# oscarknagg/voicemap

Measured on AMD Instinct MI355X. Metric: audio-sec/s embedded, 3s@16kHz siamese batch (training step), higher is better.
Workload: dtype f16; 1 GPU; siamese cfg-A train step (filters 128, embed 64, contrastive loss), 128 pairs/GPU of 3 s @ 16 kHz decimated x4 (L=12000), Adam(clipnorm 1), f16 storage; global_pairs=128, parallelism=dp1

## Files before the change

voicemap_amd/csrc/conv_wgrad.hip:

```cpp
#include "conv_common.hpp"

namespace vm {

template <typename T>
struct TnArgs {
    const T* x;
    const T* du;
    float* ws;
    int64_t x_win_stride, du_win_stride;
    int c_in, c_out, L;
    int Kk;
    int tilesI, tilesJ, splits;
    int xcd_remap;
    int64_t n_windows, win_per_split;
    int split = 0;
    int64_t tower_windows = 0;
    int splits_per_tower = 0;
    int64_t stages_per_split = 0;
};

template <typename T>
__device__ inline void split_windows(const TnArgs<T>& p, int split, int64_t& w_begin, int64_t& w_end) {
    const int tw = split / p.splits_per_tower, j = split - tw * p.splits_per_tower;
    const int64_t t0 = (int64_t)tw * p.tower_windows;
    int64_t t1 = t0 + p.tower_windows;
    if (t1 > p.n_windows) t1 = p.n_windows;
    w_begin = t0 + (int64_t)j * p.win_per_split;
    w_end = w_begin + p.win_per_split;
    if (w_end > t1) w_end = t1;
    if (w_begin > w_end) w_begin = w_end;
}

template <typename T, int PITCH, int SZ = (int)sizeof(T)> struct Transpose4;
template <typename T, int PITCH> struct Transpose4<T, PITCH, 2> {
    __device__ static inline void store(char* lds_tile, int col0, int pg, const u32x4 (&v)[4]) {
#pragma unroll
        for (int j = 0; j < 8; ++j) {
            const uint32_t sel = (j & 1) ? 0x07060302u : 0x05040100u;
            u32x2 o;
            o[0] = __builtin_amdgcn_perm(v[1][j >> 1], v[0][j >> 1], sel);
            o[1] = __builtin_amdgcn_perm(v[3][j >> 1], v[2][j >> 1], sel);
            *reinterpret_cast<u32x2*>(lds_tile + (col0 + j) * PITCH + pg * 8) = o;
        }
    }
};
template <typename T, int PITCH> struct Transpose4<T, PITCH, 4> {
    __device__ static inline void store(char* lds_tile, int col0, int pg, const u32x4 (&v)[4]) {
#pragma unroll
        for (int j = 0; j < 4; ++j) {
            u32x4 o = {v[0][j], v[1][j], v[2][j], v[3][j]};
            *reinterpret_cast<u32x4*>(lds_tile + (col0 + j) * PITCH + pg * 16) = o;
        }
    }
};

template <int PITCH>
struct Transpose4Split {
    __device__ static inline void store(char* lds_tile, int col0, int pg, const u32x4 (&v)[4]) {
#pragma unroll
        for (int j = 0; j < 4; ++j) {
            const u32x4 o = {v[0][j], v[1][j], v[2][j], v[3][j]};
            u32x2 h, l;
            split_f32x4(o, h, l);
            *reinterpret_cast<u32x2*>(lds_tile + (col0 + j) * PITCH + pg * 8) = h;
            *reinterpret_cast<u32x2*>(lds_tile + (col0 + j) * PITCH + 64 + pg * 8) = l;
        }
    }
};

template <typename T, int KB, bool SPLIT = false>
__global__ __launch_bounds__(256) void conv_tn_kernel(TnArgs<T> p) {
    static_assert(!SPLIT || (sizeof(T) == 4 && KB == 128), "split-bf16 arithmetic: fp32 storage, 128-byte stages");
    using G = Geo<KB>;
    constexpr int VEC = Elem<T>::kVec;
    constexpr int BKP = KB / (int)sizeof(T);
    constexpr int PG = BKP / 4;
    constexpr int ITEMS = (128 / VEC) * PG;
    constexpr int NIT = ITEMS / 128;
    __shared__ __attribute__((aligned(16))) char lds[2 * 2 * G::TILE];

    const int tid = threadIdx.x, lane = tid & 63, w = tid >> 6, wm = w >> 1, wn = w & 1;
    int64_t b = blockIdx.x;
    {
        const int64_t NT = (int64_t)p.tilesI * p.tilesJ;
        const int64_t full = (int64_t)(p.splits / 8) * 8 * NT;
        if (p.xcd_remap && b < full) {
            const int64_t xcd = b & 7, local = b >> 3;
            b = ((local / NT) * 8 + xcd) * NT + local % NT;
        }
    }
    const int tj = (int)(b % p.tilesJ);
    b /= p.tilesJ;
    const int ti = (int)(b % p.tilesI);
    const int split = (int)(b / p.tilesI);
    const int i0 = ti * BM, j0 = tj * BN;

    const bool is_x = tid < 128;
    const T* base0 = is_x ? p.x : p.du + p.c_out;
    const int64_t win_stride = is_x ? p.x_win_stride : p.du_win_stride;
    const int row_c = is_x ? p.c_in : p.c_out;
    const int which = is_x ? 0 : 1;
    int pg[NIT], col0[NIT], toff[NIT];
    bool col_ok[NIT];
#pragma unroll
    for (int it = 0; it < NIT; ++it) {
        const int item = (tid & 127) + it * 128;
        pg[it] = item % PG;
        col0[it] = (item / PG) * VEC;
        const int gcol = (is_x ? i0 : j0) + col0[it];
        col_ok[it] = gcol < (is_x ? p.Kk : p.c_out);
        toff[it] = pg[it] * 4 * row_c + (col_ok[it] ? gcol : 0);
    }

    int64_t w_begin, w_end;
    split_windows(p, split, w_begin, w_end);
    const int stages_per_win = (p.L + BKP - 1) / BKP;
    const int64_t n_stages = (w_end - w_begin) * stages_per_win;

    f32x16 acc[2][2];
    zero_acc(acc);

    int64_t ld_n = w_begin;
    int ld_s = 0;
    u32x4 rv[NIT][4];
    auto gload = [&]() {
        const int tb = ld_s * BKP;
        const T* wbase = base0 + ld_n * win_stride + (int64_t)tb * row_c;
#pragma unroll
        for (int it = 0; it < NIT; ++it) {
#pragma unroll
            for (int r = 0; r < 4; ++r) {
                const int t = tb + pg[it] * 4 + r;
                if (col_ok[it] && t < p.L) {
                    rv[it][r] = *reinterpret_cast<const u32x4*>(wbase + toff[it] + r * row_c);
                } else {
                    rv[it][r] = u32x4{0, 0, 0, 0};
                }
            }
        }
        if (++ld_s == stages_per_win) {
            ld_s = 0;
            ++ld_n;
        }
    };
    if (n_stages > 0) gload();
    for (int64_t st = 0; st < n_stages; ++st) {
        const int buf = (int)(st & 1);
        char* mine = lds + (buf * 2 + which) * G::TILE;
#pragma unroll
        for (int it = 0; it < NIT; ++it) {
            if constexpr (SPLIT) {
                Transpose4Split<G::PITCH>::store(mine, col0[it], pg[it], rv[it]);
            } else {
                Transpose4<T, G::PITCH>::store(mine, col0[it], pg[it], rv[it]);
            }
        }
        __syncthreads();
        if (st + 1 < n_stages) gload();
        if constexpr (SPLIT) {
            mma_slice_split<KB>(lds + (buf * 2 + 0) * G::TILE, lds + (buf * 2 + 1) * G::TILE, wm, wn, lane, acc);
        } else {
            mma_slice<T, KB>(lds + (buf * 2 + 0) * G::TILE, lds + (buf * 2 + 1) * G::TILE, wm, wn, lane, acc);
        }
    }

    float* out = p.ws + (int64_t)split * p.Kk * p.c_out;
    const int hi = lane >> 5;
#pragma unroll
    for (int im = 0; im < 2; ++im) {
        const int row = i0 + wm * 64 + im * 32 + (lane & 31);
        if (row >= p.Kk) continue;
#pragma unroll
        for (int in = 0; in < 2; ++in) {
#pragma unroll
            for (int g = 0; g < 4; ++g) {
                const int col = j0 + wn * 64 + in * 32 + 8 * g + 4 * hi;
                if (col < p.c_out) {
                    f32x4 v = {acc[im][in][4 * g], acc[im][in][4 * g + 1], acc[im][in][4 * g + 2], acc[im][in][4 * g + 3]};
                    *reinterpret_cast<f32x4*>(out + (int64_t)row * p.c_out + col) = v;
                }
            }
        }
    }
}

template <typename T, int KB, bool SPLIT = false>
__global__ __launch_bounds__(512) void conv_tn256_kernel(TnArgs<T> p) {
    static_assert(!SPLIT || (sizeof(T) == 4 && KB == 128), "split-bf16 arithmetic: fp32 storage, 128-byte stages");
    using G = Geo<KB>;
    constexpr int VEC = Elem<T>::kVec;
    constexpr int BKP = KB / (int)sizeof(T);
    constexpr int PG = BKP / 4;
    constexpr int TM = 256, TN_ = 256;
    constexpr int OPB = TM * G::PITCH;
    constexpr int KSTEPS = KB / Mfma<T>::KSTEP_BYTES;
    static_assert((TM / VEC) * PG == 512, "one item per thread and operand");
    __shared__ __attribute__((aligned(16))) char lds[2 * 2 * OPB];

    const int tid = threadIdx.x, lane = tid & 63, w = tid >> 6, wm = w >> 1, wn = w & 1;
    int64_t b = blockIdx.x;
    {
        const int64_t NT = (int64_t)p.tilesI * p.tilesJ;
        const int64_t full = (int64_t)(p.splits / 8) * 8 * NT;
        if (p.xcd_remap && b < full) {
            const int64_t xcd = b & 7, local = b >> 3;
            b = ((local / NT) * 8 + xcd) * NT + local % NT;
        }
    }
    const int tj = (int)(b % p.tilesJ);
    b /= p.tilesJ;
    const int ti = (int)(b % p.tilesI);
    const int split = (int)(b / p.tilesI);
    const int i0 = ti * TM, j0 = tj * TN_;

    const int pg = tid % PG, col0 = (tid / PG) * VEC;
    const bool x_ok = i0 + col0 < p.Kk, d_ok = j0 + col0 < p.c_out;
    const int x_toff = pg * 4 * p.c_in + (x_ok ? i0 + col0 : 0);
    const int d_toff = pg * 4 * p.c_out + (d_ok ? j0 + col0 : 0);
    const T* d_base0 = p.du + p.c_out;

    int64_t w_begin, w_end;
    split_windows(p, split, w_begin, w_end);
    const int stages_per_win = (p.L + BKP - 1) / BKP;
    const int64_t n_stages = (w_end - w_begin) * stages_per_win;

    f32x16 acc[2][4];
#pragma unroll
    for (int i = 0; i < 2; ++i)
#pragma unroll
        for (int j = 0; j < 4; ++j)
#pragma unroll
            for (int r = 0; r < 16; ++r) acc[i][j][r] = 0.f;

    int64_t ld_n = w_begin;
    int ld_s = 0;
    u32x4 rx0[4], rd0[4], rx1[4], rd1[4];
    auto gload = [&](u32x4 (&rx)[4], u32x4 (&rd)[4]) {
        const int tb = ld_s * BKP;
        const T* xb = p.x + ld_n * p.x_win_stride + (int64_t)tb * p.c_in;
        const T* db = d_base0 + ld_n * p.du_win_stride + (int64_t)tb * p.c_out;
#pragma unroll
        for (int r = 0; r < 4; ++r) {
            const bool tok = tb + pg * 4 + r < p.L;
            rx[r] = (x_ok && tok) ? *reinterpret_cast<const u32x4*>(xb + x_toff + r * p.c_in) : u32x4{0, 0, 0, 0};
            rd[r] = (d_ok && tok) ? *reinterpret_cast<const u32x4*>(db + d_toff + r * p.c_out) : u32x4{0, 0, 0, 0};
        }
        if (++ld_s == stages_per_win) {
            ld_s = 0;
            ++ld_n;
        }
    };
    const int r = lane & 31, kh = lane >> 5;
    auto step = [&](int64_t st, u32x4 (&rx)[4], u32x4 (&rd)[4]) {
        char* ta = lds + (int)(st & 1) * 2 * OPB;
        char* tb_ = ta + OPB;
        if constexpr (SPLIT) {
            Transpose4Split<G::PITCH>::store(ta, col0, pg, rx);
            Transpose4Split<G::PITCH>::store(tb_, col0, pg, rd);
        } else {
            Transpose4<T, G::PITCH>::store(ta, col0, pg, rx);
            Transpose4<T, G::PITCH>::store(tb_, col0, pg, rd);
        }
        __syncthreads();
        if (st + 2 < n_stages) gload(rx, rd);
        const char* pa = ta + (wm * 64 + r) * G::PITCH;
        const char* pb = tb_ + (wn * 128 + r) * G::PITCH;
        if constexpr (SPLIT) {
            using M = Mfma<bf16>;
#pragma unroll
            for (int s = 0; s < 2; ++s) {
                const M::Frag a0h = M::load(pa, s, kh), a1h = M::load(pa + 32 * G::PITCH, s, kh);
                const M::Frag a0l = M::load(pa, s + 2, kh), a1l = M::load(pa + 32 * G::PITCH, s + 2, kh);
#pragma unroll
                for (int in = 0; in < 4; ++in) {
                    const M::Frag bh = M::load(pb + in * 32 * G::PITCH, s, kh), bl = M::load(pb + in * 32 * G::PITCH, s + 2, kh);
                    acc[0][in] = M::run(bl, a0h, acc[0][in]);
                    acc[1][in] = M::run(bl, a1h, acc[1][in]);
                    acc[0][in] = M::run(bh, a0l, acc[0][in]);
                    acc[1][in] = M::run(bh, a1l, acc[1][in]);
                    acc[0][in] = M::run(bh, a0h, acc[0][in]);
                    acc[1][in] = M::run(bh, a1h, acc[1][in]);
                }
            }
            return;
        }
#pragma unroll
        for (int s = 0; s < KSTEPS; ++s) {
            typename Mfma<T>::Frag a0 = Mfma<T>::load(pa, s, kh), a1 = Mfma<T>::load(pa + 32 * G::PITCH, s, kh);
#pragma unroll
            for (int in = 0; in < 4; ++in) {
                typename Mfma<T>::Frag bf = Mfma<T>::load(pb + in * 32 * G::PITCH, s, kh);
                acc[0][in] = Mfma<T>::run(bf, a0, acc[0][in]);
                acc[1][in] = Mfma<T>::run(bf, a1, acc[1][in]);
            }
        }
    };
    if (n_stages > 0) gload(rx0, rd0);
    if (n_stages > 1) gload(rx1, rd1);
    for (int64_t st = 0; st < n_stages; st += 2) {
        step(st, rx0, rd0);
        if (st + 1 < n_stages) step(st + 1, rx1, rd1);
    }

    float* out = p.ws + (int64_t)split * p.Kk * p.c_out;
    const int hi = lane >> 5;
#pragma unroll
    for (int im = 0; im < 2; ++im) {
        const int row = i0 + wm * 64 + im * 32 + (lane & 31);
        if (row >= p.Kk) continue;
#pragma unroll
        for (int in = 0; in < 4; ++in) {
#pragma unroll
            for (int g = 0; g < 4; ++g) {
                const int col = j0 + wn * 128 + in * 32 + 8 * g + 4 * hi;
                if (col < p.c_out) {
                    f32x4 v = {acc[im][in][4 * g], acc[im][in][4 * g + 1], acc[im][in][4 * g + 2], acc[im][in][4 * g + 3]};
                    *reinterpret_cast<f32x4*>(out + (int64_t)row * p.c_out + col) = v;
                }
            }
        }
    }
}

namespace t8x {
constexpr int ROWS = 256;
constexpr int ABLK = ROWS * 128;
constexpr int A_BYTES = 2 * ABLK;
constexpr int BBLK = 64 * 128;
constexpr int BSTAGE = 2 * BBLK;
constexpr int LDS_BYTES = A_BYTES + 4 * BSTAGE;
struct Frag4 {
    u32x2 lo[4], hi[4];
};
}

template <typename T>
__global__ __launch_bounds__(512) void conv_tn8x_kernel(TnArgs<T> p) {
    static_assert(sizeof(T) == 2, "16-bit storage types (bf16 / f16)");
    using V8 = typename Mfma<T>::Frag;
    using namespace t8x;
    __shared__ __attribute__((aligned(1024))) char lds[LDS_BYTES];
    const int tid = threadIdx.x, lane = tid & 63;
    const int w = __builtin_amdgcn_readfirstlane(tid >> 6);
    const int wm = w >> 1, wn = w & 1;

    int64_t b = blockIdx.x;
    {
        const int64_t NT = (int64_t)p.tilesI * p.tilesJ;
        const int64_t full = (int64_t)(p.splits / 8) * 8 * NT;
        if (p.xcd_remap && b < full) {
            const int64_t xcd = b & 7, local = b >> 3;
            b = ((local / NT) * 8 + xcd) * NT + local % NT;
        }
    }
    const int tj = __builtin_amdgcn_readfirstlane((int)(b % p.tilesJ));
    b /= p.tilesJ;
    const int ti = __builtin_amdgcn_readfirstlane((int)(b % p.tilesI));
    const int split = __builtin_amdgcn_readfirstlane((int)(b / p.tilesI));
    const int ci0 = ti * 128, j0 = tj * 128;

    int w_begin, w_end;
    {
        int64_t wb, we;
        split_windows(p, split, wb, we);
        w_begin = (int)wb;
        w_end = (int)we;
    }
    const int spw = (p.L + 2 + 63) / 64;
    const int G = w_end > w_begin ? (w_end - w_begin) * spw : 0;

    f32x16 acc[3][2];
#pragma unroll
    for (int t = 0; t < 3; ++t)
#pragma unroll
        for (int j = 0; j < 2; ++j)
#pragma unroll
            for (int e = 0; e < 16; ++e) acc[t][j][e] = 0.f;

    if (G > 0) {
        for (int i = tid * 16; i < A_BYTES; i += 512 * 16) *reinterpret_cast<u32x4*>(lds + i) = u32x4{0, 0, 0, 0};
        __syncthreads();

        const int drow = w * 8 + (lane >> 3);
        const int dchunk = ((lane & 7) ^ (((lane >> 4) & 1) << 2)) * 8;
        const char* const x_base = reinterpret_cast<const char*>(p.x);
        const char* const d_base = reinterpret_cast<const char*>(p.du);
        auto stage = [&](int slot, int n, int st) {
            const int t = st * 64 + drow;
            {
                int r = t < p.L + 1 ? t : p.L + 1;
                const char* src = x_base + n * p.x_win_stride * 2;
                char* dst = lds + slot * 8192 + w * 1024;
#pragma unroll
                for (int j = 0; j < 2; ++j) {
                    int c0 = ci0 + j * 64;
                    c0 = c0 < p.c_in ? c0 : 0;
                    glds16(src + (unsigned)(r * p.c_in + c0 + dchunk) * 2u, dst + j * ABLK);
                }
            }
            {
                const int r = (t < p.L ? t : p.L) + 1;
                const char* src = d_base + n * p.du_win_stride * 2;
                char* dst = lds + A_BYTES + slot * BSTAGE + w * 1024;
#pragma unroll
                for (int j = 0; j < 2; ++j) {
                    int co0 = j0 + j * 64;
                    co0 = co0 < p.c_out ? co0 : 0;
                    glds16(src + (unsigned)(r * p.c_out + co0 + dchunk) * 2u, dst + j * BBLK);
                }
            }
        };

        const int li = lane & 15, lg = (lane >> 4) & 1, kh = lane >> 5;
        const int rowl = kh * 8 + (li >> 2);
        const int sub = lg * 32 + (li & 3) * 8;
        int a_off[3];
#pragma unroll
        for (int t = 0; t < 3; ++t) a_off[t] = (rowl + t) * 128 + (((wm & 1) ^ (((rowl + t) >> 1) & 1)) * 64) + sub;
        const int b_off = rowl * 128 + ((((rowl >> 1) & 1)) * 64) + sub;
        const uint32_t lds0 = (uint32_t)(uintptr_t)(__attribute__((address_space(3))) const char*)lds;
        auto tr_pair = [&](u32x2& lo, u32x2& hi, uint32_t a_lo, uint32_t a_hi) {
            asm volatile("ds_read_b64_tr_b16 %0, %1" : "=v"(lo) : "v"(a_lo));
            asm volatile("ds_read_b64_tr_b16 %0, %1" : "=v"(hi) : "v"(a_hi));
        };
        auto read_a = [&](Frag4& fa, int slot, int tap) {
            const uint32_t blk = lds0 + (wm >> 1) * ABLK;
            const uint32_t u = slot * 8192 + a_off[tap];
#pragma unroll
            for (int s = 0; s < 4; ++s)
                tr_pair(fa.lo[s], fa.hi[s], blk + ((u + s * 2048) & (ABLK - 1)), blk + ((u + s * 2048 + 512) & (ABLK - 1)));
        };
        auto read_b = [&](Frag4& fb, int slot, int jn) {
            const uint32_t a = lds0 + A_BYTES + slot * BSTAGE + wn * BBLK + (b_off ^ (jn * 64));
#pragma unroll
            for (int s = 0; s < 4; ++s) tr_pair(fb.lo[s], fb.hi[s], a + s * 2048, a + s * 2048 + 512);
        };
        auto opf = [](const Frag4& f, int s) {
            const u32x4 v = {f.lo[s][0], f.lo[s][1], f.hi[s][0], f.hi[s][1]};
            return __builtin_bit_cast(V8, v);
        };
        auto mma_a = [&](const Frag4& a0, const Frag4& b0, const Frag4& b1, f32x16& c0, f32x16& c1) {
            __builtin_amdgcn_s_setprio(1);
#pragma unroll
            for (int s = 0; s < 4; ++s) {
                c0 = Mfma<T>::run(opf(b0, s), opf(a0, s), c0);
                c1 = Mfma<T>::run(opf(b1, s), opf(a0, s), c1);
            }
            __builtin_amdgcn_s_setprio(0);
        };
        auto mma_b = [&](const Frag4& a0, const Frag4& a1, const Frag4& b0, const Frag4& b1, f32x16& c00, f32x16& c01, f32x16& c10,
                         f32x16& c11) {
            __builtin_amdgcn_s_setprio(1);
#pragma unroll
            for (int s = 0; s < 4; ++s) {
                c00 = Mfma<T>::run(opf(b0, s), opf(a0, s), c00);
                c01 = Mfma<T>::run(opf(b1, s), opf(a0, s), c01);
                c10 = Mfma<T>::run(opf(b0, s), opf(a1, s), c10);
                c11 = Mfma<T>::run(opf(b1, s), opf(a1, s), c11);
            }
            __builtin_amdgcn_s_setprio(0);
        };
        auto slot_end = [&]() {
            __builtin_amdgcn_sched_barrier(0);
            asm volatile("" ::: "memory");
            __builtin_amdgcn_s_barrier();
            asm volatile("" ::: "memory");
            __builtin_amdgcn_sched_barrier(0);
        };
        auto read_done = [&]() { asm volatile("s_waitcnt lgkmcnt(0)" ::: "memory"); };

        int nn = w_begin, ss = 0, staged = 0;
        auto stage_next = [&]() {
            stage(staged & 3, nn, ss);
            ++staged;
            if (++ss == spw) {
                ss = 0;
                ++nn;
            }
        };
        stage_next();
        if (G > 1) stage_next();
        if (G > 2) stage_next();

        Frag4 fa0, fa1, fb0, fb1;
        {
            if (G > 2) {
                wait_vmcnt<4>();
            } else {
                wait_vmcnt<0>();
            }
            slot_end();
            if (w >= 4) slot_end();
            for (int g = 0; g < G; ++g) {
                const int slot = g & 3;
                read_a(fa0, slot, 0);
                read_b(fb0, slot, 0);
                read_b(fb1, slot, 1);
                read_done();
                slot_end();
                mma_a(fa0, fb0, fb1, acc[0][0], acc[0][1]);
                slot_end();
                read_a(fa1, slot, 1);
                read_a(fa0, slot, 2);
                if (staged < G) {
                    stage_next();
                    wait_vmcnt<4>();
                } else {
                    wait_vmcnt<0>();
                }
                read_done();
                slot_end();
                mma_b(fa1, fa0, fb0, fb1, acc[1][0], acc[1][1], acc[2][0], acc[2][1]);
                slot_end();
            }
            if (w < 4) slot_end();
        }
    }

    float* out = p.ws + (int64_t)split * p.Kk * p.c_out;
    const int hi = lane >> 5;
    const int ci = ci0 + wm * 32 + (lane & 31);
    if (ci0 + wm * 32 < p.c_in) {
#pragma unroll
        for (int t = 0; t < 3; ++t) {
            const int64_t row = (int64_t)t * p.c_in + ci;
#pragma unroll
            for (int jn = 0; jn < 2; ++jn) {
#pragma unroll
                for (int g4 = 0; g4 < 4; ++g4) {
                    const int col = j0 + wn * 64 + jn * 32 + 8 * g4 + 4 * hi;
                    if (col < p.c_out) {
                        const f32x4 v = {acc[t][jn][4 * g4], acc[t][jn][4 * g4 + 1], acc[t][jn][4 * g4 + 2], acc[t][jn][4 * g4 + 3]};
                        *reinterpret_cast<f32x4*>(out + row * p.c_out + col) = v;
                    }
                }
            }
        }
    }
}

#ifndef VM_TN9_ABL
#define VM_TN9_ABL 0
#endif
template <typename T, bool PW>
__global__ __launch_bounds__(PW ? 768 : 512) void conv_tn9_kernel(TnArgs<T> p) {
    static_assert(sizeof(T) == 2, "16-bit storage types (bf16 / f16)");
    using V8 = typename Mfma<T>::Frag;
    using namespace t8x;
    __shared__ __attribute__((aligned(1024))) char lds[LDS_BYTES];
    const int tid = threadIdx.x, lane = tid & 63;
    const int w = __builtin_amdgcn_readfirstlane(tid >> 6);
    const int wm = w >> 1, wn = w & 1;

    int64_t b = blockIdx.x;
    {
        const int64_t NT = (int64_t)p.tilesI * p.tilesJ;
        const int64_t full = (int64_t)(p.splits / 8) * 8 * NT;
        if (p.xcd_remap && b < full) {
            const int64_t xcd = b & 7, local = b >> 3;
            b = ((local / NT) * 8 + xcd) * NT + local % NT;
        } else if (p.xcd_remap) {
            const int64_t rest = (int64_t)p.splits * NT - full, per = rest / 8, bb = b - full;
            if (bb < per * 8) b = full + (bb & 7) * per + (bb >> 3);
        }
    }
    const int tj = __builtin_amdgcn_readfirstlane((int)(b % p.tilesJ));
    b /= p.tilesJ;
    const int ti = __builtin_amdgcn_readfirstlane((int)(b % p.tilesI));
    const int split = __builtin_amdgcn_readfirstlane((int)(b / p.tilesI));
    const int ci0 = ti * 128, j0 = tj * 128;

    const int spw = (p.L + 2 + 63) / 64;
    int nn0, ss0 = 0, G, Gs;
    if (p.stages_per_split > 0) {
        const int tw = split / p.splits_per_tower, j = split - tw * p.splits_per_tower;
        const int64_t t0 = (int64_t)tw * p.tower_windows;
        int64_t t1 = t0 + p.tower_windows;
        if (t1 > p.n_windows) t1 = p.n_windows;
        const int64_t S = (t1 - t0) * spw;
        int64_t g0 = (int64_t)j * p.stages_per_split, g1 = g0 + p.stages_per_split;
        g0 = g0 < S ? g0 : S;
        g1 = g1 < S ? g1 : S;
        G = __builtin_amdgcn_readfirstlane((int)(g1 - g0));
        nn0 = __builtin_amdgcn_readfirstlane((int)(t0 + g0 / spw));
        ss0 = __builtin_amdgcn_readfirstlane((int)(g0 % spw));
        Gs = G + ((G > 0 && g1 % spw != 0) ? 1 : 0);
    } else {
        int64_t wb, we;
        split_windows(p, split, wb, we);
        nn0 = (int)wb;
        G = we > wb ? (int)(we - wb) * spw : 0;
        Gs = G;
    }

    f32x16 acc[3][2];
#pragma unroll
    for (int t = 0; t < 3; ++t)
#pragma unroll
        for (int j = 0; j < 2; ++j)
#pragma unroll
            for (int e = 0; e < 16; ++e) acc[t][j][e] = 0.f;

    if (G > 0) {
        for (int i = tid * 16; i < A_BYTES; i += (PW ? 768 : 512) * 16) *reinterpret_cast<u32x4*>(lds + i) = u32x4{0, 0, 0, 0};
        __syncthreads();

        const int dchunk = ((lane & 7) ^ (((lane >> 4) & 1) << 2)) * 8;
        const char* const x_base = reinterpret_cast<const char*>(p.x);
        const char* const d_base = reinterpret_cast<const char*>(p.du);
        auto piece_of = [&](int wr, int slot, int n, int st, int q) {
            const int t = st * 64 + wr * 8 + (lane >> 3);
            const int j = q & 1;
            if (q < 2) {
                const int r = t < p.L + 1 ? t : p.L + 1;
                int c0 = ci0 + j * 64;
                c0 = c0 < p.c_in ? c0 : 0;
                glds16(x_base + n * p.x_win_stride * 2 + (unsigned)(r * p.c_in + c0 + dchunk) * 2u, lds + slot * 8192 + wr * 1024 + j * ABLK);
            } else {
                const int r = (t < p.L ? t : p.L) + 1;
                int co0 = j0 + j * 64;
                co0 = co0 < p.c_out ? co0 : 0;
                glds16(d_base + n * p.du_win_stride * 2 + (unsigned)(r * p.c_out + co0 + dchunk) * 2u,
                       lds + A_BYTES + slot * BSTAGE + wr * 1024 + j * BBLK);
            }
        };
        auto piece = [&](int slot, int n, int st, int q) { piece_of(w, slot, n, st, q); };
        int nn = nn0, ss = ss0, staged = 0;
        auto advance = [&]() {
            ++staged;
            if (++ss == spw) {
                ss = 0;
                ++nn;
            }
        };

        const int li = lane & 15, lg = (lane >> 4) & 1, kh = lane >> 5;
        const int rowl = kh * 8 + (li >> 2);
        const int sub = lg * 32 + (li & 3) * 8;
        int a_off[3];
#pragma unroll
        for (int t = 0; t < 3; ++t) a_off[t] = (rowl + t) * 128 + (((wm & 1) ^ (((rowl + t) >> 1) & 1)) * 64) + sub;
        const int b_off = rowl * 128 + ((((rowl >> 1) & 1)) * 64) + sub;
#if defined(__HIP_DEVICE_COMPILE__)
        const uint32_t lds0 = (uint32_t)(uintptr_t)(__attribute__((address_space(3))) const char*)lds;
#else
        const uint32_t lds0 = 0;
#endif
        const uint32_t ablk = lds0 + (wm >> 1) * ABLK;
        const uint32_t bblk = lds0 + A_BYTES + wn * BBLK;

        if constexpr (PW) {
            if (w >= 8) {
                const int w0 = 2 * (w - 8);
                auto stage_all = [&]() {
#pragma unroll
                    for (int i = 0; i < 2; ++i)
#pragma unroll
                        for (int q = 0; q < 4; ++q) piece_of(w0 + i, staged & 3, nn, ss, q);
                    advance();
                };
                for (int i = 0; i < 3 && staged < Gs; ++i) stage_all();
                if (Gs > 2) {
                    wait_vmcnt<8>();
                } else {
                    wait_vmcnt<0>();
                }
                __builtin_amdgcn_s_barrier();
                for (int g = 0; g < G; ++g) {
                    if (staged < Gs) {
                        stage_all();
                        wait_vmcnt<8>();
                    } else {
                        wait_vmcnt<0>();
                    }
                    asm volatile("" ::: "memory");
                    __builtin_amdgcn_s_barrier();
                    asm volatile("" ::: "memory");
                }
                return;
            }
            __builtin_amdgcn_s_barrier();
        } else {
            for (int i = 0; i < 3 && staged < Gs; ++i) {
#pragma unroll
                for (int q = 0; q < 4; ++q) piece(staged & 3, nn, ss, q);
                advance();
            }
            if (Gs > 2) {
                wait_vmcnt<4>();
            } else {
                wait_vmcnt<0>();
            }
            __builtin_amdgcn_s_barrier();
        }

        struct Fr {
            u32x2 lo, hi;
        };
        Fr fa[2][3], fb[2][2];
#pragma unroll
        for (int t = 0; t < 3; ++t) fa[1][t].lo = fa[1][t].hi = u32x2{0u, 0u};
#pragma unroll
        for (int j = 0; j < 2; ++j) fb[1][j].lo = fb[1][j].hi = u32x2{0u, 0u};

#define VM_TR(DST, ADDR, OFF) \
    if constexpr (!(VM_TN9_ABL & 2)) asm volatile("ds_read_b64_tr_b16 %0, %1 offset:" #OFF : "=v"(DST) : "v"(ADDR))
#define VM_RDA(SET, TAP, S)                                      \
    if constexpr ((S) == 0) {                                    \
        VM_TR(fa[SET][TAP].lo, aaddr[TAP], 0);                   \
        VM_TR(fa[SET][TAP].hi, aaddr[TAP], 512);                 \
    } else if constexpr ((S) == 1) {                             \
        VM_TR(fa[SET][TAP].lo, aaddr[TAP], 2048);                \
        VM_TR(fa[SET][TAP].hi, aaddr[TAP], 2560);                \
    } else if constexpr ((S) == 2) {                             \
        VM_TR(fa[SET][TAP].lo, aaddr[TAP], 4096);                \
        VM_TR(fa[SET][TAP].hi, aaddr[TAP], 4608);                \
    } else {                                                     \
        VM_TR(fa[SET][TAP].lo, a3lo[TAP], 0);                    \
        VM_TR(fa[SET][TAP].hi, a3hi[TAP], 0);                    \
    }
#define VM_RDB(SET, JN, S)                                       \
    if constexpr ((S) == 0) {                                    \
        VM_TR(fb[SET][JN].lo, baddr[JN], 0);                     \
        VM_TR(fb[SET][JN].hi, baddr[JN], 512);                   \
    } else if constexpr ((S) == 1) {                             \
        VM_TR(fb[SET][JN].lo, baddr[JN], 2048);                  \
        VM_TR(fb[SET][JN].hi, baddr[JN], 2560);                  \
    } else if constexpr ((S) == 2) {                             \
        VM_TR(fb[SET][JN].lo, baddr[JN], 4096);                  \
        VM_TR(fb[SET][JN].hi, baddr[JN], 4608);                  \
    } else {                                                     \
        VM_TR(fb[SET][JN].lo, baddr[JN], 6144);                  \
        VM_TR(fb[SET][JN].hi, baddr[JN], 6656);                  \
    }
#define VM_LGKM(N, F) \
    if constexpr (!(VM_TN9_ABL & 2)) asm volatile("s_waitcnt lgkmcnt(" #N ")" : "+v"((F).lo), "+v"((F).hi))
#define VM_FRAG(F) __builtin_bit_cast(V8, (u32x4{(F).lo[0], (F).lo[1], (F).hi[0], (F).hi[1]}))
#define VM_MMA(SET, TAP, JN)                                                                                                   \
    if constexpr (!(VM_TN9_ABL & 8)) acc[TAP][JN] = Mfma<T>::run(VM_FRAG(fb[SET][JN]), VM_FRAG(fa[SET][TAP]), acc[TAP][JN]);   \
    else acc[TAP][JN][0] += __builtin_bit_cast(float, fb[SET][JN].lo[0] ^ fa[SET][TAP].hi[1]);                                 \
    __builtin_amdgcn_sched_barrier(0)
#define VM_KSTEP(CUR, NXT, SN, Q)                     \
    VM_LGKM(6, fb[CUR][0]);                           \
    VM_LGKM(6, fa[CUR][0]);                           \
    VM_MMA(CUR, 0, 0);                                \
    VM_RDB(NXT, 0, SN);                               \
    VM_LGKM(6, fa[CUR][1]);                           \
    VM_MMA(CUR, 1, 0);                                \
    VM_RDA(NXT, 0, SN);                               \
    VM_LGKM(6, fa[CUR][2]);                           \
    VM_MMA(CUR, 2, 0);                                \
    VM_RDA(NXT, 1, SN);                               \
    VM_LGKM(6, fb[CUR][1]);                           \
    VM_MMA(CUR, 0, 1);                                \
    VM_RDA(NXT, 2, SN);                               \
    if (!PW && more && !(VM_TN9_ABL & 1)) piece(staged & 3, nn, ss, Q); \
    __builtin_amdgcn_sched_barrier(0);                \
    VM_MMA(CUR, 1, 1);                                \
    VM_RDB(NXT, 1, SN);                               \
    VM_MMA(CUR, 2, 1)

        for (int g = 0; g < G; ++g) {
            const int slot = g & 3;
            const bool more = staged < Gs;
            uint32_t aaddr[3], a3lo[3], a3hi[3], baddr[2];
#pragma unroll
            for (int t = 0; t < 3; ++t) {
                const uint32_t u = slot * 8192 + a_off[t];
                aaddr[t] = ablk + u;
                a3lo[t] = ablk + ((u + 3 * 2048) & (ABLK - 1));
                a3hi[t] = ablk + ((u + 3 * 2048 + 512) & (ABLK - 1));
            }
#pragma unroll
            for (int j = 0; j < 2; ++j) baddr[j] = bblk + slot * BSTAGE + (b_off ^ (j * 64));
            VM_RDB(0, 0, 0);
            VM_RDA(0, 0, 0);
            VM_RDA(0, 1, 0);
            VM_RDA(0, 2, 0);
            VM_RDB(0, 1, 0);
            __builtin_amdgcn_sched_barrier(0);
            VM_MMA(1, 1, 1);
            VM_MMA(1, 2, 1);
            VM_KSTEP(0, 1, 1, 0);
            VM_KSTEP(1, 0, 2, 1);
            VM_KSTEP(0, 1, 3, 2);
            VM_LGKM(6, fb[1][0]);
            VM_LGKM(6, fa[1][0]);
            VM_MMA(1, 0, 0);
            VM_LGKM(4, fa[1][1]);
            VM_MMA(1, 1, 0);
            VM_LGKM(2, fa[1][2]);
            VM_MMA(1, 2, 0);
            VM_LGKM(0, fb[1][1]);
            VM_MMA(1, 0, 1);
            if constexpr (!PW) {
                if (more) {
                    if (!(VM_TN9_ABL & 1)) piece(staged & 3, nn, ss, 3);
                    advance();
                    if (!(VM_TN9_ABL & 1)) wait_vmcnt<4>();
                } else {
                    wait_vmcnt<0>();
                }
            }
            __builtin_amdgcn_sched_barrier(0);
            asm volatile("" ::: "memory");
            if (!(VM_TN9_ABL & 4)) __builtin_amdgcn_s_barrier();
            asm volatile("" ::: "memory");
            __builtin_amdgcn_sched_barrier(0);
        }
        VM_MMA(1, 1, 1);
        VM_MMA(1, 2, 1);
#undef VM_KSTEP
#undef VM_MMA
#undef VM_FRAG
#undef VM_LGKM
#undef VM_RDB
#undef VM_RDA
#undef VM_TR
    }

    float* out = p.ws + (int64_t)split * p.Kk * p.c_out;
    const int hi = lane >> 5;
    const int ci = ci0 + wm * 32 + (lane & 31);
    if (ci0 + wm * 32 < p.c_in) {
#pragma unroll
        for (int t = 0; t < 3; ++t) {
            const int64_t row = (int64_t)t * p.c_in + ci;
#pragma unroll
            for (int jn = 0; jn < 2; ++jn) {
#pragma unroll
                for (int g4 = 0; g4 < 4; ++g4) {
                    const int col = j0 + wn * 64 + jn * 32 + 8 * g4 + 4 * hi;
                    if (col < p.c_out) {
                        const f32x4 v = {acc[t][jn][4 * g4], acc[t][jn][4 * g4 + 1], acc[t][jn][4 * g4 + 2], acc[t][jn][4 * g4 + 3]};
                        *reinterpret_cast<f32x4*>(out + row * p.c_out + col) = v;
                    }
                }
            }
        }
    }
}

template <typename T>
__global__ void prep_weights_kernel(const float* w, int c_in, int c_out, T* wf, T* wd) {
    const int64_t total = 3LL * c_in * c_out;
    const int64_t i = (int64_t)blockIdx.x * blockDim.x + threadIdx.x;
    if (i >= total) return;
    const int co = (int)(i % c_out);
    const int64_t r = i / c_out;
    const int ci = (int)(r % c_in);
    const int k = (int)(r / c_in);
    const T v = Elem<T>::from_f(w[i]);
    wf[(int64_t)co * 3 * c_in + (int64_t)k * c_in + ci] = v;
    wd[(int64_t)ci * 3 * c_out + (int64_t)(2 - k) * c_out + co] = v;
}

}

using namespace vm;

static int tiles(int64_t x, int t) { return (int)((x + t - 1) / t); }

namespace vm {
int g_tn9 = 1;
int g_tn9_stages = 1;
int g_tn_x = 1;
int g_tn_tile = 256;
}

static bool tn_x_shape(int c_in, int c_out) { return g_tn_x && c_in % 64 == 0 && c_out % 64 == 0; }
static bool tn_use_256(int c_in, int c_out) { return g_tn_tile == 256 && 3 * c_in >= 192 && c_out >= 192; }
static bool tn_stage_splits(int c_in, int c_out) { return tn_x_shape(c_in, c_out) && g_tn9 != 0 && g_tn9_stages != 0; }
static int64_t tn9_stages_per_window(int64_t L) { return (L + 2 + 63) / 64; }

static int wgrad_splits_per_tower(int64_t n_windows, int64_t tower_windows, int64_t L, int c_in, int c_out) {
    const bool big = tn_use_256(c_in, c_out);
    const bool xres = tn_x_shape(c_in, c_out);
    const int tile = big ? 256 : 128;
    const int64_t t = xres ? (int64_t)tiles(c_in, 128) * tiles(c_out, 128) : (int64_t)tiles(3 * c_in, tile) * tiles(c_out, tile);
    const int64_t slots = (big || xres) ? 256 : 512;
    const double t_window = xres ? 2.0 * 384 * 128 * (double)L / 5.0e12 : 2.0 * tile * tile * (double)L / (big ? 4.0e12 : 1.0e12);
    const double t_slab = 8.0 * 3.0 * c_in * c_out / 3.0e12;
    const int64_t towers = (n_windows + tower_windows - 1) / tower_windows;
    if (tn_stage_splits(c_in, c_out)) {
        const int64_t spw = tn9_stages_per_window(L), S = tower_windows * spw;
        const double t_stage = t_window / (double)spw;
        int64_t best_spt = 1;
        double best = -1.0;
        for (int64_t spt = 1; spt <= S && spt <= 4096; ++spt) {
            const int64_t splits = towers * spt, sps = (S + spt - 1) / spt;
            const int64_t rounds = (t * splits + slots - 1) / slots;
            const double cost = (double)(rounds * (sps + 1)) * t_stage + (double)splits * t_slab;
            if (best < 0.0 || cost < best) {
                best = cost;
                best_spt = spt;
            }
        }
        return (int)best_spt;
    }
    int64_t best_wps = 1;
    double best_cost = -1.0;
    for (int64_t wps = 1; wps <= tower_windows; ++wps) {
        const int64_t splits = towers * ((tower_windows + wps - 1) / wps);
        const int64_t rounds = (t * splits + slots - 1) / slots;
        const double cost = (double)(rounds * wps) * t_window + (double)splits * t_slab;
        if (best_cost < 0.0 || cost < best_cost) {
            best_cost = cost;
            best_wps = wps;
        }
    }
    return (int)((tower_windows + best_wps - 1) / best_wps);
}

extern "C" int vm_conv_wgrad_splits(int64_t n_windows, int64_t L, int c_in, int c_out) {
    return wgrad_splits_per_tower(n_windows, n_windows, L, c_in, c_out);
}

extern "C" int64_t vm_conv_wgrad_workspace_bytes(int64_t n_windows, int64_t L, int c_in, int c_out) {
    return (int64_t)vm_conv_wgrad_splits(n_windows, L, c_in, c_out) * 3 * c_in * c_out * (int64_t)sizeof(float) +
           slab_sum_part_bytes(3LL * c_in * c_out);
}

static int launch_wgrad(const void* in, const void* du, int64_t n_windows, int64_t tower_windows, int64_t L, int c_in, int c_out,
                        int dtype, void* ws, hipStream_t st) {
    const int spt = wgrad_splits_per_tower(n_windows, tower_windows, L, c_in, c_out);
    const int splits = spt * (int)((n_windows + tower_windows - 1) / tower_windows);
    VM_DISPATCH_DTYPE(dtype, {
        TnArgs<T> a;
        a.x = (const T*)in;
        a.du = (const T*)du;
        a.ws = (float*)ws;
        a.x_win_stride = (L + 2) * (int64_t)c_in;
        a.du_win_stride = (L + 2) * (int64_t)c_out;
        a.c_in = c_in;
        a.c_out = c_out;
        a.L = (int)L;
        a.Kk = 3 * c_in;
        const bool big = tn_use_256(c_in, c_out);
        const bool xres = sizeof(T) == 2 && tn_x_shape(c_in, c_out) && n_windows < (1LL << 30);
        a.tilesI = xres ? tiles(c_in, 128) : tiles(3 * c_in, big ? 256 : BM);
        a.tilesJ = xres ? tiles(c_out, 128) : tiles(c_out, big ? 256 : BN);
        a.splits = splits;
        a.xcd_remap = 1;
        a.n_windows = n_windows;
        a.tower_windows = tower_windows;
        a.splits_per_tower = spt;
        a.win_per_split = (tower_windows + spt - 1) / spt;
        if (xres && tn_stage_splits(c_in, c_out)) a.stages_per_split = (tower_windows * tn9_stages_per_window(L) + spt - 1) / spt;
        a.split = dtype == VM_F32S;
        const dim3 grid((unsigned)((int64_t)splits * a.tilesI * a.tilesJ));
        if constexpr (sizeof(T) == 4) {
            if (a.split && big) {
                hipLaunchKernelGGL((conv_tn256_kernel<T, 128, true>), grid, dim3(512), 0, st, a);
            } else if (a.split) {
                hipLaunchKernelGGL((conv_tn_kernel<T, 128, true>), grid, dim3(256), 0, st, a);
            } else if (big) {
                hipLaunchKernelGGL((conv_tn256_kernel<T, 128>), grid, dim3(512), 0, st, a);
            } else {
                hipLaunchKernelGGL((conv_tn_kernel<T, 128>), grid, dim3(256), 0, st, a);
            }
        } else {
            if (xres) {
                if (g_tn9 == 2) {
                    hipLaunchKernelGGL((conv_tn9_kernel<T, true>), grid, dim3(768), 0, st, a);
                } else if (g_tn9) {
                    hipLaunchKernelGGL((conv_tn9_kernel<T, false>), grid, dim3(512), 0, st, a);
                } else {
                    hipLaunchKernelGGL((conv_tn8x_kernel<T>), grid, dim3(512), 0, st, a);
                }
            } else if (big) {
                hipLaunchKernelGGL((conv_tn256_kernel<T, 128>), grid, dim3(512), 0, st, a);
            } else {
                hipLaunchKernelGGL((conv_tn_kernel<T, 128>), grid, dim3(256), 0, st, a);
            }
        }
    });
    return splits;
}

extern "C" int vm_conv_wgrad(const void* in, const void* du, int64_t n_windows, int64_t L, int c_in, int c_out, int dtype,
                             void* ws, float* grad_w, void* stream) {
    VM_REQUIRE(in && du && ws && grad_w, "vm_conv_wgrad: null pointer");
    VM_REQUIRE(n_windows > 0 && L > 0, "vm_conv_wgrad: bad sizes");
    VM_REQUIRE(c_in % 8 == 0 && c_out % 8 == 0, "vm_conv_wgrad: channels must be multiples of 8");
    const int splits = launch_wgrad(in, du, n_windows, n_windows, L, c_in, c_out, dtype, ws, (hipStream_t)stream);
    if (splits < 0) return splits;
    int rc = check_launch("vm_conv_wgrad");
    if (rc) return rc;
    const int64_t n = 3LL * c_in * c_out;
    return slab_sum((const float*)ws, splits, n, grad_w, n, nullptr, (float*)ws + (int64_t)splits * n, (hipStream_t)stream);
}

__global__ __launch_bounds__(256) void slab_fold_kernel(const float* __restrict__ ws, int towers, int spt, int c_in, int c_out,
                                                        const float* __restrict__ scale, const float* __restrict__ shift,
                                                        const float* __restrict__ dsum, float* __restrict__ out) {
    const int64_t nel = 3LL * c_in * c_out;
    const int64_t i = (int64_t)blockIdx.x * 256 + threadIdx.x;
    if (i >= nel) return;
    const int co = (int)(i % c_out);
    const int64_t r = i / c_out;
    const int ci = (int)(r % c_in), k = (int)(r / c_in);
    double total = 0.0;
    for (int t = 0; t < towers; ++t) {
        double s0 = 0.0, s1 = 0.0;
        int j = 0;
        for (; j + 2 <= spt; j += 2) {
            s0 += (double)ws[(int64_t)(t * spt + j) * nel + i];
            s1 += (double)ws[(int64_t)(t * spt + j + 1) * nel + i];
        }
        if (j < spt) s0 += (double)ws[(int64_t)(t * spt + j) * nel + i];
        total += (double)scale[t * c_in + ci] * (s0 + s1) + (double)shift[t * c_in + ci] * (double)dsum[((int64_t)t * 3 + k) * c_out + co];
    }
    out[i] = (float)total;
}

extern "C" int64_t vm_conv_wgrad_fold_workspace_bytes(int64_t n_windows, int64_t windows_per_tower, int64_t L, int c_in, int c_out) {
    if (windows_per_tower <= 0 || n_windows <= 0) return 0;
    const int64_t splits = (int64_t)wgrad_splits_per_tower(n_windows, windows_per_tower, L, c_in, c_out) *
                           ((n_windows + windows_per_tower - 1) / windows_per_tower);
    return splits * 3 * c_in * c_out * (int64_t)sizeof(float) + 64;
}

extern "C" int vm_conv_wgrad_fold_finish(const void* ws, int64_t n_windows, int64_t windows_per_tower, int64_t L, int c_in, int c_out,
                                         const float* scale, const float* shift, const float* dsum, float* grad_w, void* stream) {
    VM_REQUIRE(ws && scale && shift && dsum && grad_w, "vm_conv_wgrad_fold_finish: null pointer");
    VM_REQUIRE(n_windows > 0 && L > 0 && windows_per_tower > 0 && n_windows % windows_per_tower == 0,
               "vm_conv_wgrad_fold_finish: n_windows must be a positive multiple of windows_per_tower");
    const int towers = (int)(n_windows / windows_per_tower);
    const int spt = wgrad_splits_per_tower(n_windows, windows_per_tower, L, c_in, c_out);
    const int64_t n = 3LL * c_in * c_out;
    hipLaunchKernelGGL(slab_fold_kernel, dim3((unsigned)cdiv(n, 256)), dim3(256), 0, (hipStream_t)stream, (const float*)ws, towers, spt,
                       c_in, c_out, scale, shift, dsum, grad_w);
    return check_launch("vm_conv_wgrad_fold_finish");
}

extern "C" int vm_conv_wgrad_fold(const void* in_e, const void* du, int64_t n_windows, int64_t windows_per_tower, int64_t L, int c_in,
                                  int c_out, int dtype, const float* scale, const float* shift, const float* dsum, void* ws,
                                  float* grad_w, void* stream) {
    VM_REQUIRE(in_e && du && ws, "vm_conv_wgrad_fold: null pointer");
    VM_REQUIRE(dsum == nullptr || (scale && shift && grad_w), "vm_conv_wgrad_fold: scale / shift / grad_w go with dsum");
    VM_REQUIRE(n_windows > 0 && L > 0 && windows_per_tower > 0 && n_windows % windows_per_tower == 0,
               "vm_conv_wgrad_fold: n_windows must be a positive multiple of windows_per_tower");
    VM_REQUIRE(c_in % 8 == 0 && c_out % 8 == 0, "vm_conv_wgrad_fold: channels must be multiples of 8");
    const int splits = launch_wgrad(in_e, du, n_windows, windows_per_tower, L, c_in, c_out, dtype, ws, (hipStream_t)stream);
    if (splits < 0) return splits;
    int rc = check_launch("vm_conv_wgrad_fold");
    if (rc || dsum == nullptr) return rc;
    return vm_conv_wgrad_fold_finish(ws, n_windows, windows_per_tower, L, c_in, c_out, scale, shift, dsum, grad_w, stream);
}

template <typename T>
__global__ __launch_bounds__(256) void fold_bn_weights_kernel(const float* __restrict__ wt, const float* __restrict__ scale,
                                                              const float* __restrict__ shift, const float* __restrict__ bias, int c_in,
                                                              int c_out, T* __restrict__ wf, T* __restrict__ wfp, float* __restrict__ hb,
                                                              float* __restrict__ ctr_out) {
    const int lane = threadIdx.x & 63, co = blockIdx.x * 4 + (threadIdx.x >> 6);
    const int t = blockIdx.y;
    if (co >= c_out) return;
    const float* sc = scale + (int64_t)t * c_in;
    const float* sh = shift + (int64_t)t * c_in;
    const int ppr = c_in / 8;
    const int nk = 3 * (c_in / 32);
    double acc[3] = {0.0, 0.0, 0.0};
    for (int idx = lane; idx < 3 * ppr; idx += 64) {
        const int k = idx / ppr, ci = (idx - k * ppr) * 8;
        const float* src = wt + ((int64_t)co * 3 + k) * c_in + ci;
        const f32x4 v0 = *reinterpret_cast<const f32x4*>(src), v1 = *reinterpret_cast<const f32x4*>(src + 4);
        const f32x4 s0 = *reinterpret_cast<const f32x4*>(sc + ci), s1 = *reinterpret_cast<const f32x4*>(sc + ci + 4);
        const f32x4 h0 = *reinterpret_cast<const f32x4*>(sh + ci), h1 = *reinterpret_cast<const f32x4*>(sh + ci + 4);
        Vec16<T> o;
        double a = 0.0;
#pragma unroll
        for (int e = 0; e < 4; ++e) {
            o.set(e, v0[e] * s0[e]);
            o.set(4 + e, v1[e] * s1[e]);
        }
#pragma unroll
        for (int e = 0; e < 4; ++e) a += (double)v0[e] * (double)h0[e];
#pragma unroll
        for (int e = 0; e < 4; ++e) a += (double)v1[e] * (double)h1[e];
        acc[0] += k == 0 ? a : 0.0;
        acc[1] += k == 1 ? a : 0.0;
        acc[2] += k == 2 ? a : 0.0;
        if (wf != nullptr) store16<T>(wf + (((int64_t)t * c_out + co) * 3 + k) * c_in + ci, o);
        if (wfp != nullptr) {
            const int chunk = ci >> 5, ks = (ci >> 4) & 1, kh = (ci >> 3) & 1;
            const int64_t piece = (((((int64_t)t * (c_out >> 6) + (co >> 6)) * nk + 3 * chunk + k) * 2 + ((co >> 5) & 1)) * 2 + ks) * 64 +
                                  kh * 32 + (co & 31);
            store16<T>(wfp + piece * 8, o);
        }
    }
#pragma unroll
    for (int k = 0; k < 3; ++k)
#pragma unroll
        for (int o = 32; o > 0; o >>= 1) acc[k] += __shfl_xor(acc[k], o, 64);
    if (lane == 0) {
        float* h = hb + (int64_t)t * 4 * c_out + co;
        const float f0 = (float)acc[0], f1 = (float)acc[1], f2 = (float)acc[2];
        h[0] = f0;
        h[c_out] = f1;
        h[2 * c_out] = f2;
        const float start = bias[co] + ((f0 + f1) + f2);
        if (ctr_out != nullptr) {
            const float ctr = (float)(T)fmaxf(start, 0.f);
            ctr_out[(int64_t)t * c_out + co] = ctr;
            h[3 * c_out] = start - ctr;
        } else {
            h[3 * c_out] = start;
        }
    }
}

extern "C" int vm_fold_bn_weights(const float* wt, const float* scale, const float* shift, const float* bias, int towers, int c_in,
                                  int c_out, int dtype, void* wf_folded, void* wf_packed, float* hb, float* ctr_out, void* stream) {
    VM_REQUIRE(wt && scale && shift && bias && hb && (wf_folded || wf_packed), "vm_fold_bn_weights: null pointer");
    VM_REQUIRE(c_in > 0 && c_out > 0 && towers > 0 && towers < 65536, "vm_fold_bn_weights: bad sizes");
    VM_REQUIRE(c_in % 8 == 0, "vm_fold_bn_weights: c_in must be a multiple of 8 (got %d)", c_in);
    VM_REQUIRE(wf_packed == nullptr || (c_in % 32 == 0 && c_out % 128 == 0),
               "vm_fold_bn_weights: the fragment-order copy needs c_in %% 32 == 0 and c_out %% 128 == 0 (vm_pack_nt_weights_supported)");
    VM_REQUIRE(dtype == VM_BF16 || dtype == VM_F16, "vm_fold_bn_weights: 16-bit storage only (VM_BF16 / VM_F16), got dtype %d", dtype);
    VM_DISPATCH_16(dtype, {
        hipLaunchKernelGGL((fold_bn_weights_kernel<T>), dim3((unsigned)cdiv(c_out, 4), (unsigned)towers), dim3(256), 0,
                           (hipStream_t)stream, wt, scale, shift, bias, c_in, c_out, (T*)wf_folded, (T*)wf_packed, hb, ctr_out);
    });
    return check_launch("vm_fold_bn_weights");
}

extern "C" int vm_prep_conv_weights(const float* w, int c_in, int c_out, int dtype, void* wf, void* wd, void* stream) {
    VM_REQUIRE(w && wf && wd, "vm_prep_conv_weights: null pointer");
    const int64_t n = 3LL * c_in * c_out;
    VM_DISPATCH_DTYPE(dtype, {
        hipLaunchKernelGGL((prep_weights_kernel<T>), dim3((unsigned)cdiv(n, 256)), dim3(256), 0, (hipStream_t)stream, w,
                           c_in, c_out, (T*)wf, (T*)wd);
    });
    return check_launch("vm_prep_conv_weights");
}

constexpr int PREP_MAX_LAYERS = 8;
struct PrepBatch {
    const float* w[PREP_MAX_LAYERS];
    void* wf[PREP_MAX_LAYERS];
    void* wd[PREP_MAX_LAYERS];
    float* wt[PREP_MAX_LAYERS];
    int c_in[PREP_MAX_LAYERS], c_out[PREP_MAX_LAYERS];
};
template <typename T>
__global__ __launch_bounds__(256) void prep_weights_batch_kernel(PrepBatch pb) {
    __shared__ float tile[32][33];
    const int l = blockIdx.y;
    const int c_in = pb.c_in[l], c_out = pb.c_out[l];
    const int ti = (c_in + 31) / 32, tj = (c_out + 31) / 32;
    if ((int)blockIdx.x >= 3 * ti * tj) return;
    const int k = blockIdx.x / (ti * tj), r = blockIdx.x - k * ti * tj;
    const int ci0 = (r / tj) * 32, co0 = (r % tj) * 32;
    const float* w = pb.w[l];
    T* wf = (T*)pb.wf[l];
    T* wd = (T*)pb.wd[l];
    float* wt = pb.wt[l];
    const int tx = threadIdx.x & 31, ty = threadIdx.x >> 5;
#pragma unroll
    for (int j = 0; j < 4; ++j) {
        const int ci = ci0 + ty + 8 * j, co = co0 + tx;
        float v = 0.f;
        if (ci < c_in && co < c_out) {
            v = w[((int64_t)k * c_in + ci) * c_out + co];
            wd[(int64_t)ci * 3 * c_out + (int64_t)(2 - k) * c_out + co] = Elem<T>::from_f(v);
        }
        tile[ty + 8 * j][tx] = v;
    }
    __syncthreads();
#pragma unroll
    for (int j = 0; j < 4; ++j) {
        const int co = co0 + ty + 8 * j, ci = ci0 + tx;
        if (ci < c_in && co < c_out) {
            const float v = tile[tx][ty + 8 * j];
            const int64_t o = (int64_t)co * 3 * c_in + (int64_t)k * c_in + ci;
            wf[o] = Elem<T>::from_f(v);
            if (wt != nullptr) wt[o] = v;
        }
    }
}

extern "C" int vm_prep_conv_weights_batch(int n_layers, const float* const* w, const int* c_in, const int* c_out, int dtype,
                                          void* const* wf, void* const* wd, float* const* wt, void* stream) {
    VM_REQUIRE(w && c_in && c_out && wf && wd, "vm_prep_conv_weights_batch: null pointer");
    VM_REQUIRE(n_layers > 0 && n_layers <= PREP_MAX_LAYERS, "vm_prep_conv_weights_batch: 1..%d layers per call (got %d)", PREP_MAX_LAYERS,
               n_layers);
    PrepBatch pb;
    int64_t most = 0;
    for (int l = 0; l < n_layers; ++l) {
        VM_REQUIRE(w[l] && wf[l] && wd[l] && c_in[l] > 0 && c_out[l] > 0, "vm_prep_conv_weights_batch: bad layer %d", l);
        pb.w[l] = w[l];
        pb.wf[l] = wf[l];
        pb.wd[l] = wd[l];
        pb.wt[l] = wt != nullptr ? wt[l] : nullptr;
        pb.c_in[l] = c_in[l];
        pb.c_out[l] = c_out[l];
        const int64_t n = 3LL * ((c_in[l] + 31) / 32) * ((c_out[l] + 31) / 32);
        most = n > most ? n : most;
    }
    VM_DISPATCH_DTYPE(dtype, {
        hipLaunchKernelGGL((prep_weights_batch_kernel<T>), dim3((unsigned)most, (unsigned)n_layers), dim3(256), 0,
                           (hipStream_t)stream, pb);
    });
    return check_launch("vm_prep_conv_weights_batch");
}
```

Before: 306,100 audio-s/s.

## Derive shifted conv taps from one A fragment via alignbit instead of three LDS reads

In the weight-gradient MFMA inner loop, the kernel previously issued three transposed LDS reads per k-step, one per conv tap, each with its own address. It now reads a single A fragment per k-step plus one extra word, and builds the tap-1 and tap-2 fragments in registers with alignbit shifts and register moves. This cuts LDS read traffic and address registers for A by roughly a factor of three. In exchange it adds VALU shift work, a changed row/offset layout and rebalanced lgkmcnt waits, which could introduce stalls or correctness risk if the layout assumptions are wrong.

```diff
diff --git a/voicemap_amd/csrc/conv_wgrad.hip b/voicemap_amd/csrc/conv_wgrad.hip
--- a/voicemap_amd/csrc/conv_wgrad.hip
+++ b/voicemap_amd/csrc/conv_wgrad.hip
@@ -635,11 +635,9 @@
         };
 
         const int li = lane & 15, lg = (lane >> 4) & 1, kh = lane >> 5;
-        const int rowl = kh * 8 + (li >> 2);
+        const int rowl = kh * 32 + (li >> 2);
         const int sub = lg * 32 + (li & 3) * 8;
-        int a_off[3];
-#pragma unroll
-        for (int t = 0; t < 3; ++t) a_off[t] = (rowl + t) * 128 + (((wm & 1) ^ (((rowl + t) >> 1) & 1)) * 64) + sub;
+        const int a_off = rowl * 128 + (((wm & 1) ^ ((rowl >> 1) & 1)) * 64) + sub;
         const int b_off = rowl * 128 + ((((rowl >> 1) & 1)) * 64) + sub;
 #if defined(__HIP_DEVICE_COMPILE__)
         const uint32_t lds0 = (uint32_t)(uintptr_t)(__attribute__((address_space(3))) const char*)lds;
@@ -697,102 +695,98 @@
         struct Fr {
             u32x2 lo, hi;
         };
-        Fr fa[2][3], fb[2][2];
-#pragma unroll
-        for (int t = 0; t < 3; ++t) fa[1][t].lo = fa[1][t].hi = u32x2{0u, 0u};
-#pragma unroll
-        for (int j = 0; j < 2; ++j) fb[1][j].lo = fb[1][j].hi = u32x2{0u, 0u};
+        Fr a0[4], ax, fb[2][2];
+#pragma unroll
+        for (int s = 0; s < 4; ++s) a0[s].lo = a0[s].hi = u32x2{0u, 0u};
+        ax.lo = ax.hi = u32x2{0u, 0u};
+#pragma unroll
+        for (int i = 0; i < 2; ++i)
+#pragma unroll
+            for (int j = 0; j < 2; ++j) fb[i][j].lo = fb[i][j].hi = u32x2{0u, 0u};
+        u32x4 d1 = {0u, 0u, 0u, 0u}, d2 = {0u, 0u, 0u, 0u};
 
 #define VM_TR(DST, ADDR, OFF) \
     if constexpr (!(VM_TN9_ABL & 2)) asm volatile("ds_read_b64_tr_b16 %0, %1 offset:" #OFF : "=v"(DST) : "v"(ADDR))
-#define VM_RDA(SET, TAP, S)                                      \
+#define VM_RD(F, ADDR, S)                                        \
     if constexpr ((S) == 0) {                                    \
-        VM_TR(fa[SET][TAP].lo, aaddr[TAP], 0);                   \
-        VM_TR(fa[SET][TAP].hi, aaddr[TAP], 512);                 \
+        VM_TR((F).lo, ADDR, 0);                                  \
+        VM_TR((F).hi, ADDR, 512);                                \
     } else if constexpr ((S) == 1) {                             \
-        VM_TR(fa[SET][TAP].lo, aaddr[TAP], 2048);                \
-        VM_TR(fa[SET][TAP].hi, aaddr[TAP], 2560);                \
+        VM_TR((F).lo, ADDR, 1024);                               \
+        VM_TR((F).hi, ADDR, 1536);                               \
     } else if constexpr ((S) == 2) {                             \
-        VM_TR(fa[SET][TAP].lo, aaddr[TAP], 4096);                \
-        VM_TR(fa[SET][TAP].hi, aaddr[TAP], 4608);                \
+        VM_TR((F).lo, ADDR, 2048);                               \
+        VM_TR((F).hi, ADDR, 2560);                               \
     } else {                                                     \
-        VM_TR(fa[SET][TAP].lo, a3lo[TAP], 0);                    \
-        VM_TR(fa[SET][TAP].hi, a3hi[TAP], 0);                    \
-    }
-#define VM_RDB(SET, JN, S)                                       \
-    if constexpr ((S) == 0) {                                    \
-        VM_TR(fb[SET][JN].lo, baddr[JN], 0);                     \
-        VM_TR(fb[SET][JN].hi, baddr[JN], 512);                   \
-    } else if constexpr ((S) == 1) {                             \
-        VM_TR(fb[SET][JN].lo, baddr[JN], 2048);                  \
-        VM_TR(fb[SET][JN].hi, baddr[JN], 2560);                  \
-    } else if constexpr ((S) == 2) {                             \
-        VM_TR(fb[SET][JN].lo, baddr[JN], 4096);                  \
-        VM_TR(fb[SET][JN].hi, baddr[JN], 4608);                  \
-    } else {                                                     \
-        VM_TR(fb[SET][JN].lo, baddr[JN], 6144);                  \
-        VM_TR(fb[SET][JN].hi, baddr[JN], 6656);                  \
-    }
+        VM_TR((F).lo, ADDR, 3072);                               \
+        VM_TR((F).hi, ADDR, 3584);                               \
+    }
+#define VM_RDA(S) VM_RD(a0[(S) & 3], aaddr, (S) & 3)
+#define VM_RDB(SET, JN, S) VM_RD(fb[SET][JN], baddr[JN], S)
 #define VM_LGKM(N, F) \
     if constexpr (!(VM_TN9_ABL & 2)) asm volatile("s_waitcnt lgkmcnt(" #N ")" : "+v"((F).lo), "+v"((F).hi))
 #define VM_FRAG(F) __builtin_bit_cast(V8, (u32x4{(F).lo[0], (F).lo[1], (F).hi[0], (F).hi[1]}))
-#define VM_MMA(SET, TAP, JN)                                                                                                   \
-    if constexpr (!(VM_TN9_ABL & 8)) acc[TAP][JN] = Mfma<T>::run(VM_FRAG(fb[SET][JN]), VM_FRAG(fa[SET][TAP]), acc[TAP][JN]);   \
-    else acc[TAP][JN][0] += __builtin_bit_cast(float, fb[SET][JN].lo[0] ^ fa[SET][TAP].hi[1]);                                 \
+#define VM_TAPS(S, NEXT)                                                                  \
+    d1 = u32x4{__builtin_amdgcn_alignbit(a0[S].lo[1], a0[S].lo[0], 16),                   \
+               __builtin_amdgcn_alignbit(a0[S].hi[0], a0[S].lo[1], 16),                   \
+               __builtin_amdgcn_alignbit(a0[S].hi[1], a0[S].hi[0], 16),                   \
+               __builtin_amdgcn_alignbit((NEXT), a0[S].hi[1], 16)};                       \
+    d2 = u32x4{a0[S].lo[1], a0[S].hi[0], a0[S].hi[1], (NEXT)}
+#define VM_MMA_(A, SET, TAP, JN)                                                                                   \
+    if constexpr (!(VM_TN9_ABL & 8)) acc[TAP][JN] = Mfma<T>::run(VM_FRAG(fb[SET][JN]), (A), acc[TAP][JN]);         \
+    else acc[TAP][JN][0] += __builtin_bit_cast(float, fb[SET][JN].lo[0] ^ __builtin_bit_cast(u32x4, (A))[3]);      \
     __builtin_amdgcn_sched_barrier(0)
-#define VM_KSTEP(CUR, NXT, SN, Q)                     \
-    VM_LGKM(6, fb[CUR][0]);                           \
-    VM_LGKM(6, fa[CUR][0]);                           \
-    VM_MMA(CUR, 0, 0);                                \
-    VM_RDB(NXT, 0, SN);                               \
-    VM_LGKM(6, fa[CUR][1]);                           \
-    VM_MMA(CUR, 1, 0);                                \
-    VM_RDA(NXT, 0, SN);                               \
-    VM_LGKM(6, fa[CUR][2]);                           \
-    VM_MMA(CUR, 2, 0);                                \
-    VM_RDA(NXT, 1, SN);                               \
-    VM_LGKM(6, fb[CUR][1]);                           \
-    VM_MMA(CUR, 0, 1);                                \
-    VM_RDA(NXT, 2, SN);                               \
+#define VM_MMA0(S, JN) VM_MMA_(VM_FRAG(a0[S]), (S) & 1, 0, JN)
+#define VM_MMA1(S, JN) VM_MMA_(__builtin_bit_cast(V8, d1), (S) & 1, 1, JN)
+#define VM_MMA2(S, JN) VM_MMA_(__builtin_bit_cast(V8, d2), (S) & 1, 2, JN)
+#define VM_KSTEP(S, W0, W1, W2, Q)                    \
+    VM_LGKM(W0, fb[(S) & 1][0]);                      \
+    VM_LGKM(W0, a0[S]);                               \
+    VM_MMA0(S, 0);                                    \
+    VM_RDB(((S) + 1) & 1, 0, (S) + 1);                \
+    VM_LGKM(W1, a0[(S) + 1]);                         \
+    VM_TAPS(S, a0[(S) + 1].lo[0]);                    \
+    VM_MMA1(S, 0);                                    \
+    if constexpr ((S) < 2) {                          \
+        VM_RDA((S) + 2);                              \
+    }                                                 \
+    VM_MMA2(S, 0);                                    \
+    VM_LGKM(W2, fb[(S) & 1][1]);                      \
+    VM_MMA0(S, 1);                                    \
+    VM_RDB(((S) + 1) & 1, 1, (S) + 1);                \
     if (!PW && more && !(VM_TN9_ABL & 1)) piece(staged & 3, nn, ss, Q); \
     __builtin_amdgcn_sched_barrier(0);                \
-    VM_MMA(CUR, 1, 1);                                \
-    VM_RDB(NXT, 1, SN);                               \
-    VM_MMA(CUR, 2, 1)
+    VM_MMA1(S, 1);                                    \
+    VM_MMA2(S, 1)
 
         for (int g = 0; g < G; ++g) {
             const int slot = g & 3;
             const bool more = staged < Gs;
-            uint32_t aaddr[3], a3lo[3], a3hi[3], baddr[2];
-#pragma unroll
-            for (int t = 0; t < 3; ++t) {
-                const uint32_t u = slot * 8192 + a_off[t];
-                aaddr[t] = ablk + u;
-                a3lo[t] = ablk + ((u + 3 * 2048) & (ABLK - 1));
-                a3hi[t] = ablk + ((u + 3 * 2048 + 512) & (ABLK - 1));
-            }
+            const uint32_t u = slot * 8192 + a_off;
+            const uint32_t aaddr = ablk + u;
+            const uint32_t axaddr = ablk + ((u + 4096) & (ABLK - 1));
+            uint32_t baddr[2];
 #pragma unroll
             for (int j = 0; j < 2; ++j) baddr[j] = bblk + slot * BSTAGE + (b_off ^ (j * 64));
             VM_RDB(0, 0, 0);
-            VM_RDA(0, 0, 0);
-            VM_RDA(0, 1, 0);
-            VM_RDA(0, 2, 0);
+            VM_RDA(0);
+            VM_RDA(1);
+            VM_TR(ax.lo, axaddr, 0);
             VM_RDB(0, 1, 0);
             __builtin_amdgcn_sched_barrier(0);
-            VM_MMA(1, 1, 1);
-            VM_MMA(1, 2, 1);
-            VM_KSTEP(0, 1, 1, 0);
-            VM_KSTEP(1, 0, 2, 1);
-            VM_KSTEP(0, 1, 3, 2);
-            VM_LGKM(6, fb[1][0]);
-            VM_LGKM(6, fa[1][0]);
-            VM_MMA(1, 0, 0);
-            VM_LGKM(4, fa[1][1]);
-            VM_MMA(1, 1, 0);
-            VM_LGKM(2, fa[1][2]);
-            VM_MMA(1, 2, 0);
+            VM_MMA1(3, 1);
+            VM_MMA2(3, 1);
+            VM_KSTEP(0, 5, 5, 4, 0);
+            VM_KSTEP(1, 4, 4, 4, 1);
+            VM_KSTEP(2, 4, 4, 2, 2);
+            VM_LGKM(2, fb[1][0]);
+            VM_LGKM(2, ax);
+            VM_MMA0(3, 0);
+            VM_TAPS(3, ax.lo[0]);
+            VM_MMA1(3, 0);
+            VM_MMA2(3, 0);
             VM_LGKM(0, fb[1][1]);
-            VM_MMA(1, 0, 1);
+            VM_MMA0(3, 1);
             if constexpr (!PW) {
                 if (more) {
                     if (!(VM_TN9_ABL & 1)) piece(staged & 3, nn, ss, 3);
@@ -808,14 +802,19 @@
             asm volatile("" ::: "memory");
             __builtin_amdgcn_sched_barrier(0);
         }
-        VM_MMA(1, 1, 1);
-        VM_MMA(1, 2, 1);
+        VM_MMA1(3, 1);
+        VM_MMA2(3, 1);
 #undef VM_KSTEP
-#undef VM_MMA
+#undef VM_MMA2
+#undef VM_MMA1
+#undef VM_MMA0
+#undef VM_MMA_
+#undef VM_TAPS
 #undef VM_FRAG
 #undef VM_LGKM
 #undef VM_RDB
 #undef VM_RDA
+#undef VM_RD
 #undef VM_TR
     }
 
```

Result: no change. 307,300 audio-s/s, median of 6 (+0.4%).
